# skaegy/ORBSLAM_MapSave

Measured on AMD Instinct MI355X. Metric: frames/sec ORB extract+match, 640×480 @1000 kp, 1/2/4/8 MI355X; % HBM roofline, higher is better.
Workload: dtype u8; 1 GPU; configs[2]: 640x480 extract (8-level pyramid, FAST-9, oct-tree, rBRIEF, 1000 kp) + brute-force Hamming match vs a 2000-kp reference frame; arith=x86, streams_per_rank=2, stream_skew=False, stage_pipeline=False, global_batch=512, nfeatures=1000, reference_kp=2007, parallelism=frame-sharded x1, no data-path collective

## Files before the change

orbslam_mapsave_amd/csrc/orbfe_match.hip:

```cpp
#include <hip/hip_runtime.h>

#include <climits>
#include <type_traits>

#include "../../include/orbfe.h"
#include "orbfe_device.hpp"

namespace orbfe {

constexpr int kHistLen = kHistoLength;

__device__ __forceinline__ int hamming_rows(const uint4* a, const uint4* b) {
    return hamming256(a[0], a[1], b[0], b[1]);
}

__global__ __launch_bounds__(256) void hamming_kernel(const uint4* a, const uint4* b, int n,
                                                      int* dist) {
    const int i = blockIdx.x * 256 + threadIdx.x;
    if (i < n) dist[i] = hamming_rows(a + 2 * i, b + 2 * i);
}

constexpr int kBfMaxRefs = 65535;
typedef int i32x4 __attribute__((ext_vector_type(4)));
typedef int i32x16 __attribute__((ext_vector_type(16)));
constexpr int kBfBlock = 256;
constexpr int kBfWords = 512 / kBfBlock;
constexpr int kBfRefs = 64;
constexpr int kBfNone = 0x7fff;

__device__ __forceinline__ uint32_t nibble01(uint32_t w, int s) {
    return ((w >> s) & 15u) * 0x204081u & 0x01010101u;
}
__device__ __forceinline__ i32x4 half01(uint32_t w, int h) {
    return i32x4{(int)nibble01(w, 16 * h), (int)nibble01(w, 16 * h + 4),
                 (int)nibble01(w, 16 * h + 8), (int)nibble01(w, 16 * h + 12)};
}
__device__ __forceinline__ int kmin(int a, int b) { return a < b ? a : b; }
__device__ __forceinline__ int kmax(int a, int b) { return a > b ? a : b; }
__device__ __forceinline__ int med3(int a, int b, int c) {
    int r;
    asm("v_med3_i32 %0, %1, %2, %3" : "=v"(r) : "v"(a), "v"(b), "v"(c));
    return r;
}
__device__ __forceinline__ constexpr int bf_pos(int mt, int e) {
    return 32 * mt + (e & 3) + 8 * (e >> 2);
}

struct BfLane {
    int tb, ts;
    int best, second;
    __device__ __forceinline__ void push(int k) {
        ts = med3(tb, ts, k);
        tb = kmin(tb, k);
    }
    __device__ __forceinline__ void close(int base) {
        const int kb = ((tb >> 6) << 16) + base + (tb & 63), ks = (ts >> 6) << 16;
        second = kmin(kmin(second, ks), kmax(best, kb));
        best = kmin(best, kb);
        tb = ts = kBfNone;
    }
};

__global__ __launch_bounds__(kBfBlock) void bf_match_kernel(
    const uint8_t* q, long long q_pitch, const int* nq_arr, int nq_cap, const uint8_t* r,
    long long r_pitch, const int* nr_arr, int* out) {
    __shared__ i32x4 tile[2][16][kBfRefs];
    const int b = blockIdx.y;
    const int nq = min(nq_arr[b], nq_cap);
    const int nr = (int)min((long long)kBfMaxRefs,
                            r_pitch >= 32 ? min((long long)nr_arr[b], r_pitch / 32) : (long long)nr_arr[b]);
    if ((int)blockIdx.x * kBfBlock >= nq) return;
    const int tid = threadIdx.x, lane = tid & 63, w = tid >> 6;
    const int col = lane & 31, h = lane >> 5;
    const int q0 = blockIdx.x * kBfBlock + w * 64;
    const uint8_t* R = r + b * r_pitch;

    i32x4 bq[2][8];
    int popc[2];
    BfLane st[2];
#pragma unroll
    for (int nt = 0; nt < 2; ++nt) {
        const int qi = q0 + 32 * nt + col;
        uint4 d0 = make_uint4(0, 0, 0, 0), d1 = d0;
        if (qi < nq) {
            const uint4* Q = reinterpret_cast<const uint4*>(q + b * q_pitch) + 2 * qi;
            d0 = Q[0];
            d1 = Q[1];
        }
        const uint32_t dw[8] = {d0.x, d0.y, d0.z, d0.w, d1.x, d1.y, d1.z, d1.w};
        int pc = 0;
#pragma unroll
        for (int c = 0; c < 8; ++c) {
            pc += __popc(dw[c]);
            const i32x4 v = half01(dw[c], h);
            bq[nt][c] = i32x4{(int)((uint32_t)v.x << 7 ^ 0x40404040u),
                              (int)((uint32_t)v.y << 7 ^ 0x40404040u),
                              (int)((uint32_t)v.z << 7 ^ 0x40404040u),
                              (int)((uint32_t)v.w << 7 ^ 0x40404040u)};
        }
        popc[nt] = pc;
        st[nt].best = st[nt].second = (256 - pc) << 16;
        st[nt].tb = st[nt].ts = kBfNone;
    }
    i32x16 pos[2];
#pragma unroll
    for (int e = 0; e < 16; ++e) {
        pos[0][e] = bf_pos(0, e);
        pos[1][e] = bf_pos(1, e);
    }

    const int lrow = tid & 63, lcp = tid >> 6;
    struct Raw { uint32_t w[kBfWords]; };
    auto fetch = [&](int t) {
        const int j = t * kBfRefs + lrow;
        const uint32_t* src = reinterpret_cast<const uint32_t*>(
            R + (long long)min(j, max(nr - 1, 0)) * 32 + 4 * kBfWords * lcp);
        Raw v;
        if constexpr (kBfWords == 2) {
            const uint2 u = *reinterpret_cast<const uint2*>(src);
            v.w[0] = j < nr ? u.x : 0u;
            v.w[1] = j < nr ? u.y : 0u;
        } else {
            v.w[0] = j < nr ? src[0] : 0u;
        }
        return v;
    };
    const int nfull = nr / kBfRefs, ntiles = (nr + kBfRefs - 1) / kBfRefs;
    if (nr) {
        const Raw v = fetch(0);
#pragma unroll
        for (int j = 0; j < kBfWords; ++j) {
            tile[0][2 * (kBfWords * lcp + j) + 0][lrow] = half01(v.w[j], 0);
            tile[0][2 * (kBfWords * lcp + j) + 1][lrow] = half01(v.w[j], 1);
        }
    }
    __syncthreads();

    Raw raw = fetch(1);
    i32x16 accp;
#pragma unroll
    for (int e = 0; e < 16; ++e) accp[e] = kBfNone;
    auto step = [&](int t, auto partial_tag) {
        constexpr bool partial = decltype(partial_tag)::value;
        const int cur = t & 1;
        const Raw raw2 = fetch(t + 2);
        const int valid = nr - t * kBfRefs - 4 * h;
        uint32_t ex[4];
        auto frag = [&](int f) { return tile[cur][2 * (f & 7) + h][32 * ((f >> 3) & 1) + col]; };
        i32x4 a = frag(0), a1 = frag(1);
#pragma unroll
        for (int p = 0; p < 4; ++p) {
            const int mt = p & 1, nt = p >> 1;
            const int pmt = (p + 3) & 1, pnt = ((p + 3) & 3) >> 1;
            i32x16 acc;
#pragma unroll
            for (int c = 0; c < 8; ++c) {
                const int f = 8 * p + c;
                i32x4 a2 = a1;
                if (f + 2 < 32) a2 = frag(f + 2);
                acc = __builtin_amdgcn_mfma_i32_32x32x32_i8(a, bq[nt][c], c ? acc : pos[mt], 0, 0, 0);
#pragma unroll
                for (int u = 0; u < 2; ++u) {
                    const int e = 2 * c + u;
                    int k = accp[e];
                    if (partial && p > 0 && bf_pos(pmt, e) >= valid) k = kBfNone;
                    st[pnt].push(k);
                }
                const int n = f * kBfWords / 4;
                if ((f * kBfWords) % 4 == 0 && n < 8 * kBfWords) {
                    ex[n & 3] = nibble01(raw.w[n >> 3], 16 * ((n >> 2) & 1) + 4 * (n & 3));
                    if ((n & 3) == 3)
                        tile[cur ^ 1][2 * kBfWords * lcp + (n >> 2)][lrow] =
                            i32x4{(int)ex[0], (int)ex[1], (int)ex[2], (int)ex[3]};
                }
                a = a1;
                a1 = a2;
                __builtin_amdgcn_sched_group_barrier(0x100, 1, 0);
                __builtin_amdgcn_sched_group_barrier(0x008, 1, 0);
                __builtin_amdgcn_sched_group_barrier(0x002, 5, 0);
                __builtin_amdgcn_sched_barrier(0);
            }
            if (p == 0) st[1].close((t - 1) * kBfRefs);
            if (p == 2) st[0].close(t * kBfRefs);
            accp = acc;
        }
        raw = raw2;
        __syncthreads();
    };
    for (int t = 0; t < nfull; ++t) step(t, std::false_type{});
    if (nfull < ntiles) step(nfull, std::true_type{});
    if (ntiles) {
        const int valid = nr - (ntiles - 1) * kBfRefs - 4 * h;
#pragma unroll
        for (int e = 0; e < 16; ++e) st[1].push(bf_pos(1, e) < valid ? accp[e] : kBfNone);
        st[1].close((ntiles - 1) * kBfRefs);
    }
    int best[2] = {st[0].best, st[1].best}, second[2] = {st[0].second, st[1].second};
#pragma unroll
    for (int nt = 0; nt < 2; ++nt) {
        const int kb = best[nt] + 4 * h, ks = second[nt];
        const int ob = __shfl_xor(kb, 32), os = __shfl_xor(ks, 32);
        second[nt] = kmin(kmin(ks, os), kmax(kb, ob));
        best[nt] = kmin(kb, ob);
    }
    const int qi = q0 + 32 * h + col;
    if (qi < nq) {
        const int kb = h ? best[1] : best[0], ks = h ? second[1] : second[0];
        const int pc = h ? popc[1] : popc[0];
        const int db = (kb >> 16) + pc;
        int* o = out + ((long long)b * nq_cap + qi) * 3;
        o[0] = db >= 256 ? -1 : (kb & 0xffff);
        o[1] = db;
        o[2] = (ks >> 16) + pc;
    }
}

#ifndef ORBFE_BF_WAVES
#define ORBFE_BF_WAVES 3
#endif
typedef int i32x8 __attribute__((ext_vector_type(8)));
typedef float f32x16 __attribute__((ext_vector_type(16)));
constexpr float kBfNoneF = 32767.f;
__device__ __forceinline__ uint32_t bits8_nib(uint32_t w, int s) {
    return nibble01(w, s) | (nibble01(w, s + 4) << 4);
}
__device__ __forceinline__ i32x4 ref_fp4(uint32_t w) {
    return i32x4{(int)(bits8_nib(w, 0) << 1), (int)(bits8_nib(w, 8) << 1),
                 (int)(bits8_nib(w, 16) << 1), (int)(bits8_nib(w, 24) << 1)};
}
__device__ __forceinline__ i32x4 qry_fp4(uint32_t w) {
    return i32x4{(int)((bits8_nib(w, 0) << 3) | 0x22222222u), (int)((bits8_nib(w, 8) << 3) | 0x22222222u),
                 (int)((bits8_nib(w, 16) << 3) | 0x22222222u), (int)((bits8_nib(w, 24) << 3) | 0x22222222u)};
}
struct BfLaneF {
    float tb, ts;
    int best, second;
    __device__ __forceinline__ void push(float k) {
        ts = __builtin_amdgcn_fmed3f(tb, ts, k);
        float m;
        asm("v_min_f32 %0, %1, %2" : "=v"(m) : "v"(tb), "v"(k));
        tb = m;
    }
    __device__ __forceinline__ void close(int base) {
        const int ib = (int)tb, is = (int)ts;
        const int kb = ((ib >> 6) << 16) + base + (ib & 63), ks = (is >> 6) << 16;
        second = kmin(kmin(second, ks), kmax(best, kb));
        best = kmin(best, kb);
        tb = ts = kBfNoneF;
    }
};
constexpr int kBfMaxTiles = (kBfMaxRefs + kBfRefs) / kBfRefs;
constexpr int kBfExpandBlocks = 64;
__global__ __launch_bounds__(512) void bf_expand_kernel(const uint8_t* r, const int* nr_arr, int nb,
                                                        i32x4* E) {
    __shared__ int s_nr;
    if (threadIdx.x == 0) s_nr = 0;
    __syncthreads();
    int m = 0;
    for (int b = threadIdx.x; b < nb; b += 512) m = max(m, nr_arr[b]);
    if (m) atomicMax(&s_nr, m);
    __syncthreads();
    const int nr = min(s_nr, kBfMaxRefs);
    const int row = threadIdx.x & 63, dw = threadIdx.x >> 6;
    for (int t = blockIdx.x; t * kBfRefs < nr; t += gridDim.x) {
        const int j = t * kBfRefs + row;
        const uint32_t w = j < nr ? reinterpret_cast<const uint32_t*>(r + (long long)j * 32)[dw] : 0u;
        E[((size_t)t * 8 + dw) * kBfRefs + row] = ref_fp4(w);
    }
}

template <bool kPre>
__device__ __forceinline__ void bf_fp4_body(
    const uint8_t* q, long long q_pitch, const int* nq_arr, int nq_cap, const uint8_t* r,
    long long r_pitch, const int* nr_arr, int* out, const i32x4* E) {
    __shared__ i32x4 tile[2][8][kBfRefs];
    const int b = blockIdx.y;
    const int nq = min(nq_arr[b], nq_cap);
    const int nr = (int)min((long long)kBfMaxRefs,
                            r_pitch >= 32 ? min((long long)nr_arr[b], r_pitch / 32) : (long long)nr_arr[b]);
    if ((int)blockIdx.x * kBfBlock >= nq) return;
    const int tid = threadIdx.x, lane = tid & 63, w = tid >> 6;
    const int col = lane & 31, h = lane >> 5;
    const int q0 = blockIdx.x * kBfBlock + w * 64;
    const uint8_t* R = r + b * r_pitch;
    i32x4 bq[2][4];
    int popc[2];
    BfLaneF st[2];
#pragma unroll
    for (int nt = 0; nt < 2; ++nt) {
        const int qi = q0 + 32 * nt + col;
        uint4 d0 = make_uint4(0, 0, 0, 0), d1 = d0;
        if (qi < nq) {
            const uint4* Q = reinterpret_cast<const uint4*>(q + b * q_pitch) + 2 * qi;
            d0 = Q[0];
            d1 = Q[1];
        }
        const uint32_t dw[8] = {d0.x, d0.y, d0.z, d0.w, d1.x, d1.y, d1.z, d1.w};
        int pc = 0;
#pragma unroll
        for (int c = 0; c < 8; ++c) pc += __popc(dw[c]);
#pragma unroll
        for (int c = 0; c < 4; ++c) bq[nt][c] = qry_fp4(dw[2 * c + h]);
        popc[nt] = pc;
        st[nt].best = st[nt].second = (256 - pc) << 16;
        st[nt].tb = st[nt].ts = kBfNoneF;
    }
    f32x16 pos[2];
#pragma unroll
    for (int e = 0; e < 16; ++e) {
        pos[0][e] = (float)bf_pos(0, e);
        pos[1][e] = (float)bf_pos(1, e);
    }
    const int lrow = tid & 63, lcp = tid >> 6;
    struct Raw { uint32_t w[kBfWords]; };
    struct RawE { i32x4 v[kBfWords]; };
    auto fetch_e = [&](int t) {
        RawE v;
#pragma unroll
        for (int j = 0; j < kBfWords; ++j) v.v[j] = E[((size_t)t * 8 + kBfWords * lcp + j) * kBfRefs + lrow];
        return v;
    };
    auto fetch = [&](int t) {
        const int j = t * kBfRefs + lrow;
        const uint32_t* src = reinterpret_cast<const uint32_t*>(
            R + (long long)min(j, max(nr - 1, 0)) * 32 + 4 * kBfWords * lcp);
        Raw v;
        if constexpr (kBfWords == 2) {
            const uint2 u = *reinterpret_cast<const uint2*>(src);
            v.w[0] = j < nr ? u.x : 0u;
            v.w[1] = j < nr ? u.y : 0u;
        } else {
            v.w[0] = j < nr ? src[0] : 0u;
        }
        return v;
    };
    const int nfull = nr / kBfRefs, ntiles = (nr + kBfRefs - 1) / kBfRefs;
    if (nr) {
        if constexpr (kPre) {
            const RawE v = fetch_e(0);
#pragma unroll
            for (int j = 0; j < kBfWords; ++j) tile[0][kBfWords * lcp + j][lrow] = v.v[j];
        } else {
            const Raw v = fetch(0);
#pragma unroll
            for (int j = 0; j < kBfWords; ++j) tile[0][kBfWords * lcp + j][lrow] = ref_fp4(v.w[j]);
        }
    }
    __syncthreads();
    using RawT = std::conditional_t<kPre, RawE, Raw>;
    auto fetch_any = [&](int t) -> RawT {
        if constexpr (kPre) {
            return fetch_e(t * kBfRefs < nr ? t : 0);
        } else {
            return fetch(t);
        }
    };
    RawT raw = fetch_any(1);
    f32x16 accp;
#pragma unroll
    for (int e = 0; e < 16; ++e) accp[e] = kBfNoneF;
    const int scale_a = 127, scale_b = 127 + 6;
    auto step = [&](int t, auto partial_tag) {
        constexpr bool partial = decltype(partial_tag)::value;
        const int cur = t & 1;
        const RawT raw2 = fetch_any(t + 2);
        const int valid = nr - t * kBfRefs - 4 * h;
        auto frag = [&](int f) { return tile[cur][2 * (f & 3) + h][32 * ((f >> 2) & 1) + col]; };
        i32x4 a = frag(0), a1 = frag(1);
#pragma unroll
        for (int p = 0; p < 4; ++p) {
            const int mt = p & 1, nt = p >> 1;
            const int pmt = (p + 3) & 1, pnt = ((p + 3) & 3) >> 1;
            f32x16 acc;
#pragma unroll
            for (int c = 0; c < 4; ++c) {
                const int f = 4 * p + c;
                i32x4 a2 = a1;
                if (f + 2 < 16) a2 = frag(f + 2);
                const i32x8 av = i32x8{a[0], a[1], a[2], a[3], 0, 0, 0, 0};
                const i32x8 bv = i32x8{bq[nt][c][0], bq[nt][c][1], bq[nt][c][2], bq[nt][c][3], 0, 0, 0, 0};
                acc = __builtin_amdgcn_mfma_scale_f32_32x32x64_f8f6f4(av, bv, c ? acc : pos[mt], 4, 4, 0,
                                                                       scale_a, 0, scale_b);
#pragma unroll
                for (int u = 0; u < 4; ++u) {
                    const int e = 4 * c + u;
                    float k = accp[e];
                    if (partial && p > 0 && bf_pos(pmt, e) >= valid) k = kBfNoneF;
                    st[pnt].push(k);
                }
                if (f % 8 == 7 && (f >> 3) < kBfWords) {
                    if constexpr (kPre)
                        tile[cur ^ 1][kBfWords * lcp + (f >> 3)][lrow] = raw.v[f >> 3];
                    else
                        tile[cur ^ 1][kBfWords * lcp + (f >> 3)][lrow] = ref_fp4(raw.w[f >> 3]);
                }
                a = a1;
                a1 = a2;
                __builtin_amdgcn_sched_group_barrier(0x100, 1, 0);
                __builtin_amdgcn_sched_group_barrier(0x008, 1, 0);
                __builtin_amdgcn_sched_group_barrier(0x002, 10, 0);
                __builtin_amdgcn_sched_barrier(0);
            }
            if (p == 0) st[1].close((t - 1) * kBfRefs);
            if (p == 2) st[0].close(t * kBfRefs);
            accp = acc;
        }
        raw = raw2;
        __syncthreads();
    };
    for (int t = 0; t < nfull; ++t) step(t, std::false_type{});
    if (nfull < ntiles) step(nfull, std::true_type{});
    if (ntiles) {
        const int valid = nr - (ntiles - 1) * kBfRefs - 4 * h;
#pragma unroll
        for (int e = 0; e < 16; ++e) st[1].push(bf_pos(1, e) < valid ? accp[e] : kBfNoneF);
        st[1].close((ntiles - 1) * kBfRefs);
    }
    int best[2] = {st[0].best, st[1].best}, second[2] = {st[0].second, st[1].second};
#pragma unroll
    for (int nt = 0; nt < 2; ++nt) {
        const int kb = best[nt] + 4 * h, ks = second[nt];
        const int ob = __shfl_xor(kb, 32), os = __shfl_xor(ks, 32);
        second[nt] = kmin(kmin(ks, os), kmax(kb, ob));
        best[nt] = kmin(kb, ob);
    }
    const int qi = q0 + 32 * h + col;
    if (qi < nq) {
        const int kb = h ? best[1] : best[0], ks = h ? second[1] : second[0];
        const int pc = h ? popc[1] : popc[0];
        const int db = (kb >> 16) + pc;
        int* o = out + ((long long)b * nq_cap + qi) * 3;
        o[0] = db >= 256 ? -1 : (kb & 0xffff);
        o[1] = db;
        o[2] = (ks >> 16) + pc;
    }
}

__global__ __launch_bounds__(kBfBlock, ORBFE_BF_WAVES) void bf_match_fp4_kernel(
    const uint8_t* q, long long q_pitch, const int* nq_arr, int nq_cap, const uint8_t* r,
    long long r_pitch, const int* nr_arr, int* out) {
    bf_fp4_body<false>(q, q_pitch, nq_arr, nq_cap, r, r_pitch, nr_arr, out, nullptr);
}
__global__ __launch_bounds__(kBfBlock, ORBFE_BF_WAVES) void bf_match_fp4e_kernel(
    const uint8_t* q, long long q_pitch, const int* nq_arr, int nq_cap, const uint8_t* r,
    long long r_pitch, const int* nr_arr, int* out, const i32x4* E) {
    bf_fp4_body<true>(q, q_pitch, nq_arr, nq_cap, r, r_pitch, nr_arr, out, E);
}

using BfKernel = void (*)(const uint8_t*, long long, const int*, int, const uint8_t*, long long,
                          const int*, int*);

struct SfiArgs {
    DevFrame f1, f2;
    const float* prev;
    float window;
    CandArgs c;
};

template <int kMode>
__global__ __launch_bounds__(256) void sfi_cand_kernel(SfiArgs a) {
    const int i1 = blockIdx.x * 4 + (threadIdx.x >> 6);
    if (i1 >= a.f1.n) return;
    const CandSink<kMode> sink{a.c, i1};
    if (!sink.room()) return;
    const orbfe_keypoint k1 = a.f1.k[i1];
    if (k1.octave > 0) return sink.finish(0);
    const uint4* d1 = a.f1.desc + 2 * i1;
    const uint4 q0 = d1[0], q1 = d1[1];
    int2* out = sink.out();
    const int n = features_in_area_wave(
        a.f2, a.prev[2 * i1], a.prev[2 * i1 + 1], a.window, k1.octave, k1.octave,
        [](int) { return true; },
        [&](int i2, int rank) {
            sink.put(out, rank, i2, [&] {
                const uint4* d2 = a.f2.desc + 2 * i2;
                return hamming256(q0, q1, d2[0], d2[1]);
            });
        });
    sink.finish(n);
}

__device__ __forceinline__ int rot_bin(float a1, float a2) {
    float rot = a1 - a2;
    if (rot < 0.0) rot += 360.0f;
    int bin = (int)roundf(rot * (1.0f / kHistLen));
    if (bin == kHistLen) bin = 0;
    return bin;
}

__host__ __device__ __forceinline__ void three_maxima(const int* h, int& i1, int& i2, int& i3) {
    int m1 = 0, m2 = 0, m3 = 0;
    i1 = i2 = i3 = -1;
    for (int i = 0; i < kHistLen; ++i) {
        const int s = h[i];
        if (s > m1) { m3 = m2; m2 = m1; m1 = s; i3 = i2; i2 = i1; i1 = i; }
        else if (s > m2) { m3 = m2; m2 = s; i3 = i2; i2 = i; }
        else if (s > m3) { m3 = s; i3 = i; }
    }
    if (m2 < 0.1f * (float)m1) { i2 = -1; i3 = -1; }
    else if (m3 < 0.1f * (float)m1) { i3 = -1; }
}

__device__ __forceinline__ int lane_id() { return threadIdx.x & 63; }

__device__ __forceinline__ int first_lane(bool pred) {
    const unsigned long long b = __ballot(pred);
    return b ? __builtin_ctzll(b) : 64;
}

constexpr int kSfiSlotK = 64;
struct SfiRoundArgs {
    int n1, n2, k;
    const int* off;
    const int2* cand;
    long long cand_cap;
    float nnratio;
    int* dec[2];
    int2* list[3];
    int* lcnt[3];
    int* chg;
    int* overflow;
    int* status;
};

__global__ __launch_bounds__(256) void sfi_init_kernel(int* dec0, int nd, int* lcnt, int nl, int* chg, int nc) {
    for (int i = blockIdx.x * 256 + threadIdx.x; i < max(nd, max(nl, nc)); i += gridDim.x * 256) {
        if (i < nd) dec0[i] = (int)0xfefefefe;
        if (i < nl) lcnt[i] = 0;
        if (i < nc) chg[i] = 0;
    }
}

__global__ __launch_bounds__(256) void sfi_round_kernel(SfiRoundArgs a, int r) {
    if (r > 0 && a.chg[r - 1] == 0) return;
    const int gid = blockIdx.x * 256 + threadIdx.x;
    if (gid < a.n2) a.lcnt[(r + 2) % 3][gid] = 0;
    const int i = blockIdx.x * 4 + (threadIdx.x >> 6);
    if (i >= a.n1) return;
    const int lane = threadIdx.x & 63;
    const int e0 = a.off[i];
    const int e1 = a.off[i + 1] > a.cand_cap ? e0 : a.off[i + 1];
    if (e1 - e0 >= 65536) {
        if (lane == 0) atomicExch(a.status, ORBFE_ERR_UNSUPPORTED);
        return;
    }
    const int2* Lr = a.list[r % 3];
    const int* Cr = a.lcnt[r % 3];
    uint32_t k1 = 0xffffffffu, k2 = 0xffffffffu;
    for (int e = e0 + lane; e < e1; e += 64) {
        const int2 c = a.cand[e];
        const int n = min(Cr[c.x], a.k);
        int md = INT_MAX;
        for (int k = 0; k < n; ++k) {
            const int2 q = Lr[(size_t)c.x * a.k + k];
            if (q.x < i) md = min(md, q.y);
        }
        if (md <= c.y) continue;
        const uint32_t key = ((uint32_t)c.y << 16) | (uint32_t)(e - e0);
        if (key < k1) { k2 = k1; k1 = key; }
        else if (key < k2) { k2 = key; }
    }
    const uint32_t best = __ockl_wfred_min_u32(k1);
    const uint32_t sec = __ockl_wfred_min_u32(k1 == best ? k2 : k1);
    const int bd = best == 0xffffffffu ? INT_MAX : (int)(best >> 16);
    const int sd = sec == 0xffffffffu ? INT_MAX : (int)(sec >> 16);
    const bool acc = bd <= kThLow && (float)bd < (float)sd * a.nnratio;
    if (lane != 0) return;
    const int d = acc ? a.cand[e0 + (int)(best & 0xffff)].x : -1;
    if (d != a.dec[r & 1][i]) a.chg[r] = 1;
    a.dec[~r & 1][i] = d;
    if (d >= 0) {
        const int p = atomicAdd(&a.lcnt[(r + 1) % 3][d], 1);
        if (p < a.k) a.list[(r + 1) % 3][(size_t)d * a.k + p] = make_int2(i, bd);
        else *a.overflow = 1;
    }
}

struct SfiFinalArgs {
    int n1, k;
    const orbfe_keypoint* k1;
    const orbfe_keypoint* k2;
    const int* dec;
    const int2* list;
    const int* lcnt;
    int check_ori;
    int* m12;
    int* rotbin;
    float* prev;
    int* nmatches;
};
__global__ __launch_bounds__(1024) void sfi_final_kernel(SfiFinalArgs a) {
    __shared__ int hist[kHistLen];
    __shared__ int top[3];
    __shared__ int nm;
    if (threadIdx.x < kHistLen) hist[threadIdx.x] = 0;
    if (threadIdx.x == 0) nm = 0;
    __syncthreads();
    for (int i = threadIdx.x; i < a.n1; i += 1024) {
        const int d = a.dec[i];
        int own = -1, bin = -1;
        if (d >= 0) {
            int last = -1;
            const int n = min(a.lcnt[d], a.k);
            for (int k = 0; k < n; ++k) last = max(last, a.list[(size_t)d * a.k + k].x);
            if (last == i) own = d;
            if (a.check_ori) {
                bin = rot_bin(a.k1[i].angle, a.k2[d].angle);
                atomicAdd(&hist[bin], 1);
            }
        }
        a.m12[i] = own;
        a.rotbin[i] = bin;
    }
    __syncthreads();
    if (a.check_ori && threadIdx.x == 0) three_maxima(hist, top[0], top[1], top[2]);
    __syncthreads();
    int cnt = 0;
    for (int i = threadIdx.x; i < a.n1; i += 1024) {
        int j = a.m12[i];
        const int b = a.rotbin[i];
        if (j >= 0 && a.check_ori && b != top[0] && b != top[1] && b != top[2]) {
            j = -1;
            a.m12[i] = -1;
        }
        if (j >= 0) {
            ++cnt;
            a.prev[2 * i] = a.k2[j].x;
            a.prev[2 * i + 1] = a.k2[j].y;
        }
    }
    cnt = wave_sum(cnt);
    if ((threadIdx.x & 63) == 0 && cnt) atomicAdd(&nm, cnt);
    __syncthreads();
    if (threadIdx.x == 0) *a.nmatches = nm;
}

struct SbpMps {
    int m;
    const uint8_t* in_view;
    const uint8_t* bad;
    const float* px;
    const float* py;
    const float* pxr;
    const int* lvl;
    const float* vcos;
    const uint4* desc;
    const int* nobs;
};

struct SbpLocalArgs {
    DevFrame f;
    SbpMps mp;
    const float* scale;
    float th;
    int nlevels;
    int* status;
    CandArgs c;
};

template <int kMode>
__global__ __launch_bounds__(256) void sbp_local_cand_kernel(SbpLocalArgs a) {
    const int i = blockIdx.x * 4 + (threadIdx.x >> 6);
    if (i >= a.mp.m) return;
    const CandSink<kMode> sink{a.c, i};
    if (!a.mp.in_view[i] || a.mp.bad[i]) return sink.finish(0);
    const int pl = a.mp.lvl[i];
    if (pl < 0 || pl >= a.nlevels) {
        if (a.status && (threadIdx.x & 63) == 0) atomicExch(a.status, ORBFE_ERR_UNSUPPORTED);
        return sink.finish(0);
    }
    float r = a.mp.vcos[i] > 0.998 ? 2.5f : 4.0f;
    if (a.th != 1.0) r *= a.th;
    const float rs = r * a.scale[pl];
    const float pxr = a.mp.pxr[i];
    if (!sink.room()) return;
    const uint4 q0 = a.mp.desc[2 * i], q1 = a.mp.desc[2 * i + 1];
    int2* out = sink.out();
    const int n = features_in_area_wave(
        a.f, a.mp.px[i], a.mp.py[i], rs, pl - 1, pl,
        [&](int idx) {
            return !(a.f.ur && a.f.ur[idx] > 0 && fabsf(pxr - a.f.ur[idx]) > r * a.scale[pl]);
        },
        [&](int idx, int rank) {
            sink.put(out, rank, idx, [&] {
                const uint4* d = a.f.desc + 2 * idx;
                return hamming256(q0, q1, d[0], d[1]) | (a.f.k[idx].octave << 16);
            });
        });
    sink.finish(n);
}

struct SbpLastArgs {
    DevFrame cur;
    int n_last;
    const orbfe_keypoint* lk;
    const uint8_t* valid;
    const uint8_t* outlier;
    const float* xyz;
    const uint4* desc;
    float T[12];
    float fx, fy, cx, cy, bf;
    float minx, maxx, miny, maxy;
    const float* scale;
    float th;
    int mode;
    CandArgs c;
};

template <int kMode>
__global__ __launch_bounds__(256) void sbp_last_cand_kernel(SbpLastArgs a) {
    const int i = blockIdx.x * 4 + (threadIdx.x >> 6);
    if (i >= a.n_last) return;
    const CandSink<kMode> sink{a.c, i};
    const bool room = sink.room();
    const bool live = a.valid[i] && !a.outlier[i];
    const float P[3] = {a.xyz[3 * i], a.xyz[3 * i + 1], a.xyz[3 * i + 2]};
    const int o = a.lk[i].octave;
    if (!room) return;
    int n = 0;
    {
        float pc[3];
        pose_apply(a.T, P, pc);
        const float invz = (float)(1.0 / (double)pc[2]);
        const float u = a.fx * pc[0] * invz + a.cx;
        const float v = a.fy * pc[1] * invz + a.cy;
        if (live && !(invz < 0) && !(u < a.minx || u > a.maxx) && !(v < a.miny || v > a.maxy)) {
            const float radius = a.th * a.scale[o];
            const int lo = a.mode == 0 ? o - 1 : a.mode == 1 ? o : 0;
            const int hi = a.mode == 0 ? o + 1 : a.mode == 1 ? -1 : o;
            const uint4 q0 = a.desc[2 * i], q1 = a.desc[2 * i + 1];
            int2* out = sink.out();
            const float ur = u - a.bf * invz;
            n = features_in_area_wave(
                a.cur, u, v, radius, lo, hi,
                [&](int i2) { return !(a.cur.ur && a.cur.ur[i2] > 0 && fabsf(ur - a.cur.ur[i2]) > radius); },
                [&](int i2, int rank) {
                    sink.put(out, rank, i2, [&] {
                        const uint4* d = a.cur.desc + 2 * i2;
                        return hamming256(q0, q1, d[0], d[1]);
                    });
                });
        }
    }
    sink.finish(n);
}

struct SbpKfArgs {
    DevFrame cur;
    int n;
    const uint8_t* valid;
    const uint8_t* bad;
    const uint8_t* found;
    const float* xyz;
    const float* mind;
    const float* maxd;
    const uint4* desc;
    float T[12];
    float ow[3];
    float fx, fy, cx, cy;
    float minx, maxx, miny, maxy;
    const float* scale;
    int nlevels;
    float log_scale, th;
    int* status;
    CandArgs c;
};

template <int kMode>
__global__ __launch_bounds__(256) void sbp_kf_cand_kernel(SbpKfArgs a) {
    const int i = blockIdx.x * 4 + (threadIdx.x >> 6);
    if (i >= a.n) return;
    const CandSink<kMode> sink{a.c, i};
    const bool room = sink.room();
    const bool live = a.valid[i] && !a.bad[i] && !a.found[i];
    const float P[3] = {a.xyz[3 * i], a.xyz[3 * i + 1], a.xyz[3 * i + 2]};
    const float maxd = a.maxd[i], mind = a.mind[i];
    if (!room) return;
    int n = 0;
    {
        float pc[3];
        pose_apply(a.T, P, pc);
        const float invz = (float)(1.0 / (double)pc[2]);
        const float u = a.fx * pc[0] * invz + a.cx;
        const float v = a.fy * pc[1] * invz + a.cy;
        const float po0 = P[0] - a.ow[0], po1 = P[1] - a.ow[1], po2 = P[2] - a.ow[2];
        const float dist = (float)sqrt((double)po0 * po0 + (double)po1 * po1 + (double)po2 * po2);
        const float dmax = kMaxDistInvariance * maxd, dmin = kMinDistInvariance * mind;
        const bool ok = live && !(u < a.minx || u > a.maxx) && !(v < a.miny || v > a.maxy) &&
                        !(dist < dmin || dist > dmax);
        if (ok) {
            const int lvl = predict_level(maxd, dist, a.log_scale);
            if (level_in_pyramid(lvl, a.nlevels, a.status)) {
                const float radius = a.th * a.scale[lvl];
                const uint4 q0 = a.desc[2 * i], q1 = a.desc[2 * i + 1];
                int2* out = sink.out();
                n = features_in_area_wave(
                    a.cur, u, v, radius, lvl - 1, lvl + 1, [](int) { return true; },
                    [&](int i2, int rank) {
                        sink.put(out, rank, i2, [&] {
                            const uint4* d = a.cur.desc + 2 * i2;
                            return hamming256(q0, q1, d[0], d[1]);
                        });
                    });
            }
        }
    }
    sink.finish(n);
}

constexpr int kDdBlock = 256;
constexpr int kDdStage = 64;
__global__ __launch_bounds__(kDdBlock) void distinctive_kernel(int n_mp, const int* off,
                                                               const uint4* desc, int* best,
                                                               uint4* desc_out) {
    __shared__ uint4 s_d[kDdBlock / 64][2 * kDdStage];
    const int wid = threadIdx.x >> 6, lane = threadIdx.x & 63;
    const int mp = blockIdx.x * (kDdBlock / 64) + wid;
    if (mp >= n_mp) return;
    const int o = off[mp], N = off[mp + 1] - o;
    if (N <= 0) {
        if (lane == 0) best[mp] = -1;
        return;
    }
    const uint4* d = desc + 2 * (size_t)o;
    const bool staged = N <= kDdStage;
    if (staged) {
        for (int k = lane; k < 2 * N; k += 64) s_d[wid][k] = d[k];
        __builtin_amdgcn_wave_barrier();
        __builtin_amdgcn_fence(__ATOMIC_RELEASE, "wavefront");
    }
    const uint4* src = staged ? s_d[wid] : d;
    const int k = (int)(0.5 * (double)(N - 1));
    uint32_t key = 0xffffffffu;
    for (int i = lane; i < N; i += 64) {
        const uint4 a0 = src[2 * i], a1 = src[2 * i + 1];
        int lo = 0, hi = 256;
        while (lo < hi) {
            const int mid = (lo + hi) >> 1;
            int c = 0;
            for (int j = 0; j < N; ++j) c += hamming256(a0, a1, src[2 * j], src[2 * j + 1]) <= mid;
            if (c > k) hi = mid; else lo = mid + 1;
        }
        key = min(key, ((uint32_t)lo << 16) | (uint32_t)i);
    }
#pragma unroll
    for (int s = 32; s > 0; s >>= 1) key = min(key, (uint32_t)__shfl_xor((int)key, s, 64));
    const int bi = (int)(key & 0xffff);
    if (lane == 0) best[mp] = bi;
    if (desc_out && lane < 2) desc_out[2 * (size_t)mp + lane] = d[2 * bi + lane];
}

struct FrustumArgs {
    int n;
    const float* xyz;
    const float* normal;
    const float* mind;
    const float* maxd;
    float T[12];
    float ow[3];
    float fx, fy, cx, cy, bf;
    float minx, maxx, miny, maxy, log_scale, cos_limit;
    uint8_t* in_view;
    float* px;
    float* py;
    float* pxr;
    int* lvl;
    float* vcos;
    const uint8_t* skip;
    const uint8_t* bad;
    int* n_in_view;
};

struct FrustumOut {
    float u, ur, v, vc;
    int lvl;
};
__device__ uint8_t g_zero_u8;
__device__ __forceinline__ bool frustum_eval(const FrustumArgs& a, int i, FrustumOut& o) {
    const uint8_t sk = *(a.skip ? a.skip + i : &g_zero_u8);
    const uint8_t bd = *(a.bad ? a.bad + i : &g_zero_u8);
    const float* P = a.xyz + 3 * i;
    const float* nv = a.normal + 3 * i;
    const float P0 = P[0], P1 = P[1], P2 = P[2];
    const float n0 = nv[0], n1 = nv[1], n2 = nv[2];
    const float maxd = a.maxd[i], mind = a.mind[i];
    const float Pv[3] = {P0, P1, P2};
    float pc[3];
    pose_apply(a.T, Pv, pc);
    const float invz = 1.0f / pc[2];
    const float u = a.fx * pc[0] * invz + a.cx;
    const float v = a.fy * pc[1] * invz + a.cy;
    const float dmax = kMaxDistInvariance * maxd, dmin = kMinDistInvariance * mind;
    const float po0 = P0 - a.ow[0], po1 = P1 - a.ow[1], po2 = P2 - a.ow[2];
    const float dist = (float)sqrt((double)po0 * po0 + (double)po1 * po1 + (double)po2 * po2);
    const double dot = (double)po0 * n0 + (double)po1 * n1 + (double)po2 * n2;
    const float vc = (float)(dot / dist);
    const bool in = !sk && !bd && !(pc[2] < 0.0f) && !(u < a.minx || u > a.maxx) &&
                    !(v < a.miny || v > a.maxy) && !(dist < dmin || dist > dmax) && !(vc < a.cos_limit);
    if (!in) return false;
    o.lvl = predict_level(maxd, dist, a.log_scale);
    o.u = u;
    o.ur = u - a.bf * invz;
    o.v = v;
    o.vc = vc;
    return true;
}

__device__ __forceinline__ bool frustum_point(const FrustumArgs& a, int i) {
    FrustumOut o;
    const bool in = frustum_eval(a, i, o);
    a.in_view[i] = in ? 1 : 0;
    if (!in) return false;
    a.px[i] = o.u;
    a.pxr[i] = o.ur;
    a.py[i] = o.v;
    a.lvl[i] = o.lvl;
    a.vcos[i] = o.vc;
    return true;
}

__global__ __launch_bounds__(256) void frustum_kernel(FrustumArgs a) {
    const int i = blockIdx.x * 256 + threadIdx.x;
    bool in = false;
    if (i < a.n) in = frustum_point(a, i);
    if (a.n_in_view) {
        const unsigned long long b = __ballot(in);
        if ((threadIdx.x & 63) == 0 && b) atomicAdd(a.n_in_view, __popcll(b));
    }
}

}
```

Measured before the change: 373,600 frames/s.

## Replace serial top-2 push chain with tree reduction using biased integer-min keys

Adds a positive bias to the MFMA accumulator keys so the float values can be compared as integers, and replaces the 16-step sequential min/med3 push per accumulator with a tree of 3-way top-2 merges (min3/med3). It also reorders the tile loop so both m-tiles for a given query n-tile are processed consecutively, and changes fragment prefetching to an explicit register array. The intent is to shorten the VALU dependency chain interleaved between MFMAs. The cost is higher register pressure and a more complex close/bias bookkeeping that could break correctness at the edges.

Result: faster. 381,000 frames/s, median of 6 (+2.0%).

```diff
diff --git a/orbslam_mapsave_amd/csrc/orbfe_match.hip b/orbslam_mapsave_amd/csrc/orbfe_match.hip
--- a/orbslam_mapsave_amd/csrc/orbfe_match.hip
+++ b/orbslam_mapsave_amd/csrc/orbfe_match.hip
@@ -220,7 +220,8 @@
 #endif
 typedef int i32x8 __attribute__((ext_vector_type(8)));
 typedef float f32x16 __attribute__((ext_vector_type(16)));
-constexpr float kBfNoneF = 32767.f;
+constexpr int kBfBias = 64 * 256;
+constexpr float kBfNoneF = 65535.f;
 __device__ __forceinline__ uint32_t bits8_nib(uint32_t w, int s) {
     return nibble01(w, s) | (nibble01(w, s + 4) << 4);
 }
@@ -232,21 +233,33 @@
     return i32x4{(int)((bits8_nib(w, 0) << 3) | 0x22222222u), (int)((bits8_nib(w, 8) << 3) | 0x22222222u),
                  (int)((bits8_nib(w, 16) << 3) | 0x22222222u), (int)((bits8_nib(w, 24) << 3) | 0x22222222u)};
 }
+__device__ __forceinline__ float kminf(float a, float b) {
+    return __int_as_float(kmin(__float_as_int(a), __float_as_int(b)));
+}
+__device__ __forceinline__ float kmin3f(float a, float b, float c) { return kminf(kminf(a, b), c); }
+struct BfPairF {
+    float b, s;
+};
+__device__ __forceinline__ BfPairF bf_top2(float x, float y, float z) {
+    return {kmin3f(x, y, z), __builtin_amdgcn_fmed3f(x, y, z)};
+}
+__device__ __forceinline__ BfPairF bf_merge3(BfPairF x, BfPairF y, BfPairF z) {
+    return {kmin3f(x.b, y.b, z.b), kminf(__builtin_amdgcn_fmed3f(x.b, y.b, z.b), kmin3f(x.s, y.s, z.s))};
+}
+__device__ __forceinline__ BfPairF bf_merge2(BfPairF x, BfPairF y) {
+    return {kminf(x.b, y.b), __builtin_amdgcn_fmed3f(x.b, y.b, kminf(x.s, y.s))};
+}
+__device__ __forceinline__ BfPairF bf_push(BfPairF x, float k) {
+    return {kminf(x.b, k), __builtin_amdgcn_fmed3f(x.b, x.s, k)};
+}
 struct BfLaneF {
-    float tb, ts;
+    BfPairF t;
     int best, second;
-    __device__ __forceinline__ void push(float k) {
-        ts = __builtin_amdgcn_fmed3f(tb, ts, k);
-        float m;
-        asm("v_min_f32 %0, %1, %2" : "=v"(m) : "v"(tb), "v"(k));
-        tb = m;
-    }
     __device__ __forceinline__ void close(int base) {
-        const int ib = (int)tb, is = (int)ts;
+        const int ib = (int)t.b, is = (int)t.s;
         const int kb = ((ib >> 6) << 16) + base + (ib & 63), ks = (is >> 6) << 16;
         second = kmin(kmin(second, ks), kmax(best, kb));
         best = kmin(best, kb);
-        tb = ts = kBfNoneF;
     }
 };
 constexpr int kBfMaxTiles = (kBfMaxRefs + kBfRefs) / kBfRefs;
@@ -302,14 +315,14 @@
 #pragma unroll
         for (int c = 0; c < 4; ++c) bq[nt][c] = qry_fp4(dw[2 * c + h]);
         popc[nt] = pc;
-        st[nt].best = st[nt].second = (256 - pc) << 16;
-        st[nt].tb = st[nt].ts = kBfNoneF;
+        st[nt].best = st[nt].second = (512 - pc) << 16;
+        st[nt].t = {kBfNoneF, kBfNoneF};
     }
     f32x16 pos[2];
 #pragma unroll
     for (int e = 0; e < 16; ++e) {
-        pos[0][e] = (float)bf_pos(0, e);
-        pos[1][e] = (float)bf_pos(1, e);
+        pos[0][e] = (float)(kBfBias + bf_pos(0, e));
+        pos[1][e] = (float)(kBfBias + bf_pos(1, e));
     }
     const int lrow = tid & 63, lcp = tid >> 6;
     struct Raw { uint32_t w[kBfWords]; };
@@ -365,28 +378,41 @@
         const int cur = t & 1;
         const RawT raw2 = fetch_any(t + 2);
         const int valid = nr - t * kBfRefs - 4 * h;
-        auto frag = [&](int f) { return tile[cur][2 * (f & 3) + h][32 * ((f >> 2) & 1) + col]; };
-        i32x4 a = frag(0), a1 = frag(1);
+        auto frag = [&](int g) { return tile[cur][2 * (g & 3) + h][32 * (g >> 2) + col]; };
+        i32x4 fr[8];
+        fr[0] = frag(0);
+        fr[1] = frag(1);
 #pragma unroll
         for (int p = 0; p < 4; ++p) {
-            const int mt = p & 1, nt = p >> 1;
-            const int pmt = (p + 3) & 1, pnt = ((p + 3) & 3) >> 1;
+            const int mt = p >> 1, nt = p & 1;
+            const int pmt = ((p + 3) & 3) >> 1, pnt = (p + 3) & 1;
             f32x16 acc;
+            auto key = [&](int e) {
+                return partial && p > 0 && bf_pos(pmt, e) >= valid ? kBfNoneF : accp[e];
+            };
+            BfPairF ru{}, rv{}, rw{};
+            if (p == 0) st[0].close((t - 1) * kBfRefs);
 #pragma unroll
             for (int c = 0; c < 4; ++c) {
                 const int f = 4 * p + c;
-                i32x4 a2 = a1;
-                if (f + 2 < 16) a2 = frag(f + 2);
+                const int rd = f < 2 ? f + 2 : (f >= 5 && f <= 8) ? f - 1 : -1;
+                if (rd >= 0) fr[rd] = frag(rd);
+                const i32x4 a = fr[4 * mt + c];
                 const i32x8 av = i32x8{a[0], a[1], a[2], a[3], 0, 0, 0, 0};
                 const i32x8 bv = i32x8{bq[nt][c][0], bq[nt][c][1], bq[nt][c][2], bq[nt][c][3], 0, 0, 0, 0};
                 acc = __builtin_amdgcn_mfma_scale_f32_32x32x64_f8f6f4(av, bv, c ? acc : pos[mt], 4, 4, 0,
                                                                        scale_a, 0, scale_b);
-#pragma unroll
-                for (int u = 0; u < 4; ++u) {
-                    const int e = 4 * c + u;
-                    float k = accp[e];
-                    if (partial && p > 0 && bf_pos(pmt, e) >= valid) k = kBfNoneF;
-                    st[pnt].push(k);
+                if (c == 0) {
+                    ru = bf_top2(key(0), key(1), key(2));
+                    rv = bf_top2(key(3), key(4), key(5));
+                } else if (c == 1) {
+                    ru = bf_merge3(ru, rv, bf_top2(key(6), key(7), key(8)));
+                } else if (c == 2) {
+                    rv = bf_top2(key(9), key(10), key(11));
+                    rw = bf_top2(key(12), key(13), key(14));
+                } else {
+                    ru = bf_push(bf_merge3(ru, rv, rw), key(15));
+                    st[pnt].t = pmt ? bf_merge2(st[pnt].t, ru) : ru;
                 }
                 if (f % 8 == 7 && (f >> 3) < kBfWords) {
                     if constexpr (kPre)
@@ -394,15 +420,12 @@
                     else
                         tile[cur ^ 1][kBfWords * lcp + (f >> 3)][lrow] = ref_fp4(raw.w[f >> 3]);
                 }
-                a = a1;
-                a1 = a2;
-                __builtin_amdgcn_sched_group_barrier(0x100, 1, 0);
+                if (rd >= 0) __builtin_amdgcn_sched_group_barrier(0x100, 1, 0);
                 __builtin_amdgcn_sched_group_barrier(0x008, 1, 0);
                 __builtin_amdgcn_sched_group_barrier(0x002, 10, 0);
                 __builtin_amdgcn_sched_barrier(0);
             }
             if (p == 0) st[1].close((t - 1) * kBfRefs);
-            if (p == 2) st[0].close(t * kBfRefs);
             accp = acc;
         }
         raw = raw2;
@@ -413,7 +436,8 @@
     if (ntiles) {
         const int valid = nr - (ntiles - 1) * kBfRefs - 4 * h;
 #pragma unroll
-        for (int e = 0; e < 16; ++e) st[1].push(bf_pos(1, e) < valid ? accp[e] : kBfNoneF);
+        for (int e = 0; e < 16; ++e) st[1].t = bf_push(st[1].t, bf_pos(1, e) < valid ? accp[e] : kBfNoneF);
+        st[0].close((ntiles - 1) * kBfRefs);
         st[1].close((ntiles - 1) * kBfRefs);
     }
     int best[2] = {st[0].best, st[1].best}, second[2] = {st[0].second, st[1].second};
@@ -427,7 +451,7 @@
     const int qi = q0 + 32 * h + col;
     if (qi < nq) {
         const int kb = h ? best[1] : best[0], ks = h ? second[1] : second[0];
-        const int pc = h ? popc[1] : popc[0];
+        const int pc = (h ? popc[1] : popc[0]) - 256;
         const int db = (kb >> 16) + pc;
         int* o = out + ((long long)b * nq_cap + qi) * 3;
         o[0] = db >= 256 ? -1 : (kb & 0xffff);
```
